# C-bowman/inference-tools

Hardware: AMD Instinct MI355X
Metric: GpRegressor fit+predict wall-time and GFLOP/s at N=16384, d=8; % fp64 MFMA peak (higher is better)
Workload: dtype f64

## Files before the change

### inference-tools_amd/csrc/api.hip

```cpp
#include "api_internal.h"
#include <malloc.h>


thread_local std::string g_create_err;


int lane_streams(gpmi_ctx* c, Lane& L) {
  const size_t index = c->lanes.size() - 1;
  L.owns_stream = index < 2;
  if (!L.owns_stream) L.stream = c->lanes[index % 2].stream;
  if (L.owns_stream) HIPCHK(c, hipStreamCreateWithFlags(&L.stream, hipStreamNonBlocking));
  hipDeviceProp_t prop;
  HIPCHK(c, hipGetDeviceProperties(&prop, c->device));
  c->ncu = prop.multiProcessorCount;
  HIPCHK(c, hipEventCreateWithFlags(&L.ev_la, hipEventDisableTiming));
  HIPCHK(c, hipEventCreateWithFlags(&L.ev_panel, hipEventDisableTiming));
  HIPCHK(c, hipEventCreateWithFlags(&L.ev_join, hipEventDisableTiming));
  HIPCHK(c, hipEventCreateWithFlags(&L.ev_main, hipEventDisableTiming));
  HIPCHK(c, hipEventCreateWithFlags(&L.ev_slice, hipEventDisableTiming));
  return GPMI_OK;
}


bool ensure_masked_pair(gpmi_ctx* c, Lane& L, int k) {
  (void)c;
  return L.sp[k] != nullptr && L.su[k] != nullptr;
}


int lane_masked_streams(gpmi_ctx* c, Lane& L) {
  const int ncu = c->ncu;
  if (ncu < 64 || ncu % 32 != 0) return GPMI_OK;
  for (int k = 0; k < GPMI_NPAIRS; ++k) {
    if (const char* e = std::getenv("GPMI_PANEL_CUS")) {
      const int v = std::atoi(e);
      if (v >= 8 && v <= ncu / 2 && v % 8 == 0) c->pair_cus[k] = v;
    }
    std::vector<uint32_t> panel((size_t)ncu / 32, 0u), upd((size_t)ncu / 32, 0xffffffffu);
    for (int i = 0; i < c->pair_cus[k]; ++i) {
      panel[(size_t)i / 32] |= 1u << (i % 32);
      upd[(size_t)i / 32] &= ~(1u << (i % 32));
    }
    hipError_t e1 = hipExtStreamCreateWithCUMask(&L.sp[k], (uint32_t)panel.size(), panel.data());
    hipError_t e2 = e1 == hipSuccess ? hipExtStreamCreateWithCUMask(&L.su[k], (uint32_t)upd.size(), upd.data()) : e1;
    if (e1 != hipSuccess || e2 != hipSuccess) {
      static bool told = false;
      if (!told) {
        told = true;
        std::fprintf(stderr, "[gpmi] a CU-masked stream pair could not be created (%s): this evaluation lane runs without "
                             "look-ahead and without the flag-ordered tail\n", hipGetErrorString(e1 != hipSuccess ? e1 : e2));
      }
      if (L.sp[k]) (void)hipStreamDestroy(L.sp[k]);
      if (L.su[k]) (void)hipStreamDestroy(L.su[k]);
      L.sp[k] = L.su[k] = nullptr;
      (void)hipGetLastError();
    }
  }
  return GPMI_OK;
}



int lane_alloc(gpmi_ctx* c, Lane& L) {
  if (int rc = lane_streams(c, L)) return rc;
  if (c->lanes.size() == 1 && c->np >= 40 * GPMI_NB)
    if (int rc = lane_masked_streams(c, L)) return rc;
  if (c->lanes.size() == 2 && c->np >= 40 * GPMI_NB) {
    for (int k = 0; k < GPMI_NPAIRS; ++k) {
      L.sp[k] = c->lanes[0].sp[k];
      L.su[k] = c->lanes[0].su[k];
    }
    L.owns_pair = false;
  }
  const int64_t nt = c->np / GPMI_NB;
  HIPCHK(c, hipMalloc(&L.A, sizeof(double) * c->np * c->ld));
  HIPCHK(c, hipMalloc(&L.invD, sizeof(double) * nt * GPMI_NB * GPMI_NB));
  ZERO_SYNC(c, L.invD, sizeof(double) * nt * GPMI_NB * GPMI_NB);
  HIPCHK(c, hipMalloc(&L.vec, sizeof(double) * 4 * c->np));
  HIPCHK(c, hipMalloc(&L.red, sizeof(double) * 2 * RED_SLOTS));
  HIPCHK(c, hipMalloc(&L.info, sizeof(int) * RED_SLOTS));
  HIPCHK(c, hipHostMalloc(&L.h_red, sizeof(double) * 2 * RED_SLOTS));
  HIPCHK(c, hipHostMalloc(&L.h_info, sizeof(int) * RED_SLOTS));
  return GPMI_OK;
}

#define DBG_FREE(msg) do { if (std::getenv("GPMI_DEBUG_FREE")) std::fprintf(stderr, "[free] %s\n", msg); } while (0)
void lane_free(Lane& L) {
  DBG_FREE("lane: sync main stream");
  if (L.stream) (void)hipStreamSynchronize(L.stream);
  DBG_FREE("lane: sync masked streams");
  if (!L.owns_pair)
    for (int k = 0; k < GPMI_NPAIRS; ++k) L.sp[k] = L.su[k] = nullptr;
  for (int k = 0; k < GPMI_NPAIRS; ++k) {
    if (L.sp[k]) (void)hipStreamSynchronize(L.sp[k]);
    if (L.su[k]) (void)hipStreamSynchronize(L.su[k]);
  }
  potrf_flow_free(L);
  DBG_FREE("lane: destroy events");
  if (L.ev_la) (void)hipEventDestroy(L.ev_la);
  if (L.ev_panel) (void)hipEventDestroy(L.ev_panel);
  if (L.ev_join) (void)hipEventDestroy(L.ev_join);
  if (L.ev_main) (void)hipEventDestroy(L.ev_main);
  if (L.ev_slice) (void)hipEventDestroy(L.ev_slice);
  DBG_FREE("lane: destroy masked streams");
  if (L.sp[0] || L.su[0]) {
    static const int pause_ms = [] {
      const char* e = std::getenv("GPMI_DESTROY_PAUSE_MS");
      return e ? std::atoi(e) : 50;
    }();
    std::this_thread::sleep_for(std::chrono::milliseconds(pause_ms));
  }
  for (int k = 0; k < GPMI_NPAIRS; ++k) {
    if (L.sp[k]) (void)hipStreamDestroy(L.sp[k]);
    if (L.su[k]) (void)hipStreamDestroy(L.su[k]);
  }
  DBG_FREE("lane: free buffers");
  if (L.A) (void)hipFree(L.A);
  if (L.B2) (void)hipFree(L.B2);
  if (L.inv2) (void)hipFree(L.inv2);
  if (L.inv2_t) (void)hipFree(L.inv2_t);
  if (L.gws) (void)hipFree(L.gws);
  if (L.invD) (void)hipFree(L.invD);
  if (L.vec) (void)hipFree(L.vec);
  if (L.red) (void)hipFree(L.red);
  if (L.info) (void)hipFree(L.info);
  if (L.h_red) (void)hipHostFree(L.h_red);
  if (L.h_info) (void)hipHostFree(L.h_info);
  DBG_FREE("lane: destroy main stream");
  if (L.stream && L.owns_stream) (void)hipStreamDestroy(L.stream);
  DBG_FREE("lane: done");
  L = Lane();
}

int ensure_lanes(gpmi_ctx* c, size_t count) {
  while (c->lanes.size() < count) {
    c->lanes.emplace_back();
    int rc = lane_alloc(c, c->lanes.back());
    if (rc != GPMI_OK) {
      lane_free(c->lanes.back());
      c->lanes.pop_back();
      return rc;
    }
  }
  return GPMI_OK;
}

void linv_free(LinvState& S);

void free_batch_ws(gpmi_ctx* c) {
  for (double** q : {&c->bA, &c->bInv, &c->bVec, &c->bRed, &c->bMu, &c->bB2, &c->bGws, &c->bGout, &c->bLoo, &c->bQ, &c->bNoise,
                     &c->bMixG, &c->bMixH, &c->bMixW, &c->bMixExtra}) {
    if (*q) (void)hipFree(*q);
    *q = nullptr;
  }
  for (void* q : {(void*)c->bMixP, (void*)c->bInfo, (void*)c->bParams, (void*)c->bSum})
    if (q) (void)hipFree(q);
  c->bMixP = nullptr;
  c->bInfo = nullptr;
  c->bParams = nullptr;
  c->bSum = nullptr;
  for (void* q : {(void*)c->h_bGout, (void*)c->h_bRed, (void*)c->h_bInfo})
    if (q) (void)hipHostFree(q);
  c->h_bGout = c->h_bRed = nullptr;
  c->h_bInfo = nullptr;
  c->bcap = c->bgrad_cap = c->bgrad_ntheta = c->bLoo_cap = c->bNoise_cap = c->bMix_cap = c->bQ_cap = 0;
}

void free_data(gpmi_ctx* c) {
  linv_free(c->linv);
  for (double** q : {&c->mix_g, &c->mix_scratch, &c->mix_zero, &c->Q3}) {
    if (*q) (void)hipFree(*q);
    *q = nullptr;
  }
  c->mix_nk = 0;
  c->q3_cap = 0;
// ... 763 lines not shown
```

### inference-tools_amd/csrc/gpmi_internal.h

```cpp
#pragma once
#include <hip/hip_runtime.h>
#include <cstdint>
#include <string>
#include <vector>

#include "gpmi.h"

constexpr int GPMI_NB = 128;
constexpr int GPMI_MAX_D = 64;
constexpr int GPMI_INFO_FLOW_TIMEOUT = -6;
constexpr int GPMI_NPAIRS = 1;

typedef double d2_t __attribute__((ext_vector_type(2)));
typedef double d4_t __attribute__((ext_vector_type(4)));

static inline int64_t round_up(int64_t v, int64_t m) { return (v + m - 1) / m * m; }

struct KParams {
  int kernel;
  int d;
  double a2;
  double kappa;
  double extra_diag;
  double inv_l2[GPMI_MAX_D];
// ... 16 lines not shown
constexpr int GPMI_MAX_SUM = 4;
struct CovParams : KParams {
  int nk = 0;
  KParams comp[GPMI_MAX_SUM] = {};
  CovParams() : KParams{} {}
  explicit CovParams(const KParams& k) : KParams(k) {}
};

struct ProfSlot {
  hipEvent_t e0, e1;
  int klass;
  double flops, bytes;
};

struct Lane {
  hipStream_t stream = nullptr;
  bool owns_stream = true;
  hipStream_t sp[GPMI_NPAIRS] = {nullptr};
  hipStream_t su[GPMI_NPAIRS] = {nullptr};
  bool owns_pair = true;
  struct EarlyWork {
    bool pending = false;
    const double* y = nullptr;
    const double* mu = nullptr;
    double mu_const = 0.0;
    double* r = nullptr;
    int64_t n = 0, np = 0;
    double* fill[2] = {nullptr, nullptr};
    double* ident = nullptr;
    int64_t ident_ld = 0;
  } early;
  bool identity_ready = false;
  bool pair_checked = false;
  hipEvent_t ev_la = nullptr, ev_panel = nullptr, ev_join = nullptr, ev_main = nullptr, ev_slice = nullptr;
  double* A = nullptr;
  double* invD = nullptr;
  double* B2 = nullptr;
  double* inv2 = nullptr;
  double* inv2_t = nullptr;
  bool inv2_valid = false;
  double* gws = nullptr;
  int64_t gws_doubles = 0;
  double* vec = nullptr;
  double* red = nullptr;
  int* info = nullptr;
  double* h_red = nullptr;
  int* h_info = nullptr;
  void* flow_tasks = nullptr;
  int* flow_off = nullptr;
  int* flow_flags = nullptr;
  int flow_m = 0, flow_nwg = 0, flow_nlists = 0;
  int64_t flow_ntasks = 0;
  double flow_flops_update = 0.0, flow_flops_trsm = 0.0;
};

struct LinvState {
  int64_t m = 0, mp = 0, ldm = 0;
  double* A = nullptr;
  double* At = nullptr;
  double* y = nullptr;
  double* sig2 = nullptr;
  double* zero = nullptr;
  double* K = nullptr;
  double* T = nullptr;
  double* J = nullptr;
  double* J2 = nullptr;
  double* Q = nullptr;
  double* X = nullptr;
  double* invD = nullptr;
  double* inv2 = nullptr;
  double* inv2_t = nullptr;
  double* panel = nullptr;
  double* vec = nullptr;
  double* gws = nullptr;
  int64_t gws_doubles = 0;
};

struct KdeState;
struct gpmi_sgp;

struct gpmi_ctx {
  int device = 0;
  int ncu = 256;
  int pair_cus[GPMI_NPAIRS] = {32};
  std::string err;
  int64_t n = 0, d = 0, np = 0, ld = 0;
  double* x = nullptr;
  double* y = nullptr;
  double* noise = nullptr;
  double* ycov = nullptr;
  std::vector<Lane> lanes;
  bool fitted = false;
  bool lockstep_always = false;
  bool no_flow = false;
  int64_t reserve = 0;
  CovParams fit_params;
  int sum_nk = 0;
  int sum_kinds[GPMI_MAX_SUM] = {};
  double* alpha = nullptr;
  double* Q = nullptr;
  double* Q2 = nullptr;
  int64_t mq_cap = 0;
  double* pts = nullptr;
  double* pvec = nullptr;
  double* trsm_panel = nullptr;
  int64_t trsm_panel_rows = 0;
  double* h_stage = nullptr;
// ... 146 lines not shown
struct BatchShape {
  int count = 1;
  int64_t sMat = 0;
  int64_t sInv = 0;
  int64_t sVec = 0;
};

constexpr int GPMI_MAX_MIX = 4;
void launch_scale_add(hipStream_t s, double* dst, int64_t ldd, const double* src, int64_t lds,
                      const double* gr, const double* gc, int64_t rows, int64_t cols, bool accumulate, int batch = 1,
                      int64_t sD = 0, int64_t sS = 0, int64_t sG = 0);
void launch_add_diag_vec(hipStream_t s, double* A, int64_t ld, const double* noise, double extra, int64_t n,
                         int batch = 1, int64_t sA = 0, const double* extras = nullptr);
void launch_vec_mul(hipStream_t s, const double* a, const double* b, double* out, int64_t n, int batch = 1,
                    int64_t sA = 0, int64_t sB = 0, int64_t sOut = 0);
void launch_mix_rowsum(hipStream_t s, const double* iK, const double* Km, int64_t ld, const double* alpha,
                       const double* g, double* h, int64_t n, int batch = 1, int64_t sMat = 0, int64_t sAlpha = 0,
                       int64_t sG = 0, const double* u = nullptr, int64_t sU = 0, int64_t pair = 0);

enum GemmTiles { TILES_RECT = 0, TILES_LOWER = 1 };
enum GemmOp { OP_SUB = 0, OP_ASSIGN = 1 };
void launch_gemm_nt(hipStream_t s, GemmTiles tiles, GemmOp op, double* C, int64_t ldc,
                    const double* A, int64_t lda, const double* B, int64_t ldb, int ntr, int ntc,
                    int k, unsigned long long* stamp = nullptr, const GemmBatch& bt = GemmBatch());

int64_t gemm_split_point(int64_t T, int ncu, int k);
bool gemm_mixed_launches();
void launch_gemm_nt_split(hipStream_t s, GemmTiles tiles, GemmOp op, double* C, int64_t ldc, const double* A,
                          int64_t lda, const double* B, int64_t ldb, int ntr, int ntc, int k, int64_t nfull,
                          unsigned long long* stamp = nullptr, unsigned long long* stamp_rest = nullptr,
                          int64_t nend = -1);
void launch_gemm_nt_range(hipStream_t s, GemmTiles tiles, GemmOp op, double* C, int64_t ldc, const double* A,
                          int64_t lda, const double* B, int64_t ldb, int ntr, int ntc, int k, int64_t first,
                          int64_t count, unsigned long long* stamp = nullptr);

void launch_gemm(hipStream_t s, GemmTiles tiles, GemmOp op, bool b_kmajor, int kskip, double* C,
                 int64_t ldc, const double* A, int64_t lda, const double* B, int64_t ldb, int ntr,
                 int ntc, int k, unsigned long long* stamp = nullptr, const GemmBatch& bt = GemmBatch());

hipStream_t potrf_first_update_stream(gpmi_ctx* c, Lane& lane, int64_t np, bool allow_lookahead);
void potrf_pair_quiesce(Lane& lane);
void launch_potrf_diag(hipStream_t s, double* Ablk, int64_t ld, double* invD, int* info, int col0,
                       unsigned long long* dbg = nullptr, const BatchShape& bs = BatchShape(), int* pub = nullptr,
                       int pub_val = 0);
void launch_potrf_diag_fault(hipStream_t s, double* Ablk, int64_t ld, const BatchShape& bs = BatchShape());
void potrf_lower_batched(gpmi_ctx* c, hipStream_t s, double* A, int64_t np, int64_t ld, double* invD,
                         int* info, const BatchShape& bs);
void launch_kbuild_square_batched(hipStream_t s, int kernel, const KParams* pdev, int batch, const double* x,
                                  int64_t n, int64_t np, const double* noise, double* A, int64_t ld,
                                  int64_t stride, int d, int64_t noise_stride = 0);
void potrf_lower(gpmi_ctx* c, Lane& lane, double* A, int64_t np, int64_t ld, double* invD,
                 int* info, bool allow_lookahead = true);

bool potrf_flow_enabled(gpmi_ctx* c, Lane& lane, int m);
bool potrf_flow_tail(gpmi_ctx* c, Lane& lane, double* A, int64_t ld, double* invD, int* info, int nt, int t0);
void potrf_flow_free(Lane& lane);

void trsv_forward(gpmi_ctx* c, hipStream_t s, const double* L, int64_t np, int64_t ld,
                  const double* invD, const double* r, double* out, int* err = nullptr,
                  const BatchShape& bs = BatchShape(), bool prefilled = false);
void trsv_backward(gpmi_ctx* c, hipStream_t s, const double* L, int64_t np, int64_t ld,
                   const double* invD, const double* r, double* out, int* err = nullptr,
                   const BatchShape& bs = BatchShape(), bool prefilled = false);
void lane_run_early(Lane& lane, hipStream_t s);
void trsm_identity_batched(hipStream_t s, const double* L, int64_t np, int64_t ld, const double* invD, double* Q,
                           const BatchShape& bs);
constexpr int GPMI_OB = 512;
void build_inv2(hipStream_t s, const double* L, int64_t np, int64_t ld, const double* invD, double* inv2,
                double* tmp);
void trsm_rows_forward(gpmi_ctx* c, hipStream_t s, const double* L, int64_t np, int64_t ld,
                       const double* inv2, double* Q, int64_t mp, bool upper_rhs, double* Qout,
                       double* panel);
void launch_set_identity(hipStream_t s, double* Q, int64_t ld, int64_t np, int batch = 1, int64_t sMat = 0);
void launch_copy(hipStream_t s, const double* src, double* dst, int64_t n);
void launch_copy_rows(hipStream_t s, const double* src, int64_t spitch, double* dst, int64_t dpitch, int64_t width,
                      int64_t height);
void launch_residual(hipStream_t s, const double* y, const double* mu, double mu_const, double* r,
                     int64_t n, int64_t np);
void launch_residual_batched(hipStream_t s, const double* y, const double* mus, const double* mu_consts,
                             double* r, int64_t n, int64_t np, const BatchShape& bs);
void launch_lml_reduce(hipStream_t s, const double* v, const double* L, int64_t ld, int64_t np,
                       double* red, const BatchShape& bs = BatchShape());
void launch_rows_dot(hipStream_t s, const double* Q, int64_t ld, int64_t mp, int64_t np,
                     const double* a, double* out, int batch = 1, int64_t sQ = 0, int64_t sVec = 0);
void launch_rows_sumsq(hipStream_t s, const double* Q, int64_t ld, int64_t mp, int64_t np,
                       double base, double* out, int batch = 1, int64_t sQ = 0, int64_t sVec = 0, double sign = 1.0);

void trsm_rows_backward(gpmi_ctx* c, hipStream_t s, const double* L, int64_t np, int64_t ld,
                        const double* invD, double* Q, int64_t mp, const double* inv2 = nullptr, double* panel = nullptr);

void launch_sd_reduce(hipStream_t s, const KParams& p, const double* x, int64_t n, const double* pts,
                      int64_t m, const double* Kq, int64_t ld, const double* W, int64_t ldw,
                      double scale, double* out);
void launch_grad_rhs(hipStream_t s, const KParams& p, const double* x, int64_t n, int64_t np,
                     const double* pts, int64_t rows_valid, int64_t rows_padded, const double* Kq,
                     int64_t ld, double* G);
void launch_grad_cov(hipStream_t s, const KParams& p, const double* G, int64_t ld, int64_t np,
                     int64_t m, double* cov);
```

### inference-tools_amd/csrc/potrf.hip

```cpp
#include <cstdlib>
#include <type_traits>
#include <utility>
#include <vector>

#include "gpmi_internal.h"
#include "potrf_diag.h"

namespace {

constexpr int NB = GPMI_NB;
using potrf_diag::DIAG_THREADS;

__global__ __launch_bounds__(DIAG_THREADS) void potrf_diag_kernel(double* __restrict__ A, int64_t ld,
                                                         double* __restrict__ invD,
                                                         int* __restrict__ info, int col0,
                                                         unsigned long long* __restrict__ dbg,
                                                         int64_t strideA, int64_t strideInv, int* pub, int pub_val) {
  if (pub && threadIdx.x == 0 && blockIdx.z == 0)
    __hip_atomic_store(pub, pub_val, __ATOMIC_RELAXED, __HIP_MEMORY_SCOPE_AGENT);
  __shared__ potrf_diag::DiagShared sh;
  potrf_diag::potrf_diag_body<false>(A + (int64_t)blockIdx.z * strideA, ld, invD + (int64_t)blockIdx.z * strideInv,
                                     info + blockIdx.z, col0, dbg, sh, potrf_diag::DiagPub());
}

}

namespace {
__global__ void fault_scale_kernel(double* A, int64_t ld, double f, int64_t strideA) {
  A += (int64_t)blockIdx.z * strideA;
  const int r = blockIdx.x, c = threadIdx.x;
  if (c <= r) A[(int64_t)r * ld + c] *= f;
}
}

void launch_potrf_diag_fault(hipStream_t s, double* Ablk, int64_t ld, const BatchShape& bs) {
  static const double fault = [] {
    const char* e = std::getenv("GPMI_FAULT_DIAG_EPS");
    return e ? std::atof(e) : 0.0;
  }();
  if (fault != 0.0)
    hipLaunchKernelGGL(fault_scale_kernel, dim3(NB, 1, (unsigned)bs.count), dim3(NB), 0, s, Ablk, ld, 1.0 + fault,
                       bs.sMat);
}

void launch_potrf_diag(hipStream_t s, double* Ablk, int64_t ld, double* invD, int* info, int col0,
                       unsigned long long* dbg, const BatchShape& bs, int* pub, int pub_val) {
  hipLaunchKernelGGL(potrf_diag_kernel, dim3(1, 1, (unsigned)bs.count), dim3(DIAG_THREADS), 0, s, Ablk, ld, invD,
                     info, col0, dbg, bs.sMat, bs.sInv, pub, pub_val);
  launch_potrf_diag_fault(s, Ablk, ld, bs);
}

namespace {

void factor_panel(gpmi_ctx* c, hipStream_t sp, double* A, int64_t ld, double* invD, int* info, int nt,
                  int J, int Je, int ncu = 0) {
  GemmBatch on;
  on.ncu_hint = ncu;
  on.b_lower_tri = true;
  static const bool trace = std::getenv("GPMI_CHAIN_TRACE") != nullptr;
  auto slot = [&](int tag) { return trace ? prof_stamp_slot(c, 0.0, 0.0, GPMI_PROF_NCLASS + tag) : nullptr; };
  for (int j = J; j < Je; ++j) {
    double* Ajj = A + (int64_t)j * NB * ld + (int64_t)j * NB;
    double* invDj = invD + (int64_t)j * NB * NB;
    const int below = nt - j - 1;
    {
      ProfScope ps(c, sp, GPMI_PROF_PANEL, (double)NB * NB * NB / 3.0 + 2.0 * below * NB * NB * NB,
                   8.0 * NB * NB * (2.0 + 2.0 * below));
      launch_potrf_diag(sp, Ajj, ld, invDj, info, j * NB, slot(0));
      if (below > 0) {
        double* A21 = Ajj + (int64_t)NB * ld;
        launch_gemm_nt(sp, TILES_RECT, OP_ASSIGN, A21, ld, A21, ld, invDj, NB, below, 1, NB, slot(1), on);
      }
    }
    const int pc = Je - j - 1;
    if (below > 0 && pc > 0) {
      double* A21 = Ajj + (int64_t)NB * ld;
      double* C = A21 + NB;
      const double tiles = pc * (pc + 1) / 2.0 + (double)(below - pc) * pc;
      ProfScope ps(c, sp, GPMI_PROF_PANEL, tiles * 2.0 * NB * NB * NB, tiles * 16.0 * NB * NB);
      launch_gemm_nt(sp, TILES_LOWER, OP_SUB, C, ld, A21, ld, A21, ld, below, pc, NB, slot(2));
    }
  }
}

void update_columns(gpmi_ctx* c, hipStream_t s, double* A, int64_t ld, int nt, int t0, int t1, int ka, int ke,
                    int ncu, int64_t slice = 0) {
  const int rows = nt - t0, cols = t1 - t0;
  const int kw = (ke - ka) * NB;
  if (rows <= 0 || cols <= 0 || kw <= 0) return;
  double* P = A + (int64_t)t0 * NB * ld + (int64_t)ka * NB;
  double* C = A + (int64_t)t0 * NB * ld + (int64_t)t0 * NB;
  const int64_t tiles = (int64_t)cols * (cols + 1) / 2 + (int64_t)(rows - cols) * cols - slice;
  const int64_t nfull = gemm_split_point(tiles, ncu, kw);
  static const int64_t BIG_MIN = [] {
    const char* e = std::getenv("GPMI_BIG_MIN");
    return (int64_t)(e ? std::atoi(e) : 384);
  }();
  const bool big = tiles >= BIG_MIN && kw > 128;
  int64_t nmain = big ? nfull : 0;
  if (big && nfull > 0 && nfull < tiles && gemm_mixed_launches()) nmain = tiles;
  unsigned long long* stamp = nullptr;
  unsigned long long* stamp_rest = nullptr;
  if (nmain > 0)
    stamp = prof_stamp_slot(c, (double)nmain * 2.0 * NB * NB * kw, (double)nmain * 16.0 * NB * NB + 8.0 * rows * NB * kw);
  if (tiles > nmain)
    stamp_rest = prof_stamp_slot(c, (double)(tiles - nmain) * 2.0 * NB * NB * kw, (double)(tiles - nmain) * 16.0 * NB * NB,
                                 GPMI_PROF_SYRK_REST);
  if (big)
    launch_gemm_nt_split(s, TILES_LOWER, OP_SUB, C, ld, P, ld, P, ld, rows, cols, kw, nfull, stamp, stamp_rest, tiles);
  else
    launch_gemm_nt_split(s, TILES_LOWER, OP_SUB, C, ld, P, ld, P, ld, rows, cols, kw, nfull, stamp_rest, nullptr, tiles);
}

void update_slice(gpmi_ctx* c, hipStream_t s, double* A, int64_t ld, int nt, int t0, int t1, int ka, int ke,
                  int64_t slice) {
  const int rows = nt - t0, cols = t1 - t0;
  const int kw = (ke - ka) * NB;
  double* P = A + (int64_t)t0 * NB * ld + (int64_t)ka * NB;
  double* C = A + (int64_t)t0 * NB * ld + (int64_t)t0 * NB;
  const int64_t tiles = (int64_t)cols * (cols + 1) / 2 + (int64_t)(rows - cols) * cols;
  unsigned long long* stamp =
      prof_stamp_slot(c, (double)slice * 2.0 * NB * NB * kw, (double)slice * 16.0 * NB * NB + 8.0 * rows * NB * kw,
                      GPMI_PROF_SYRK_SLICE);
  launch_gemm_nt_range(s, TILES_LOWER, OP_SUB, C, ld, P, ld, P, ld, rows, cols, kw, tiles - slice, slice, stamp);
}

int64_t slice_tiles(int rem, int64_t tiles_la, int64_t tiles_main, int kw, int ncu_main, int ncu_panel) {
  static const int PCT = [] {
    const char* e = std::getenv("GPMI_SLICE_PCT");
    return e ? std::atoi(e) : 100;
  }();
  if (PCT <= 0 || kw != 4 * NB) return 0;
  const double tile_us = 64.4 * 2.0;
  const double per_main = tile_us / (2.0 * ncu_main), per_panel = tile_us / (2.0 * ncu_panel);
  static const double CHAIN0 = [] {
    const char* e = std::getenv("GPMI_SLICE_CHAIN_US");
    return e ? std::atof(e) : 146.0;
  }();
  static const double SLOPE = [] {
    const char* e = std::getenv("GPMI_SLICE_CHAIN_SLOPE");
    return e ? std::atof(e) : 6.1;
  }();
  const double chain = CHAIN0 + SLOPE * rem;
  const double su = 20.0 + (double)(tiles_la + tiles_main) * per_main;
  double x = (su - chain) / (per_main + per_panel) * PCT / 100.0;
  const int64_t round = 2 * ncu_panel;
  int64_t n = x > 0 ? (int64_t)(x / round) * round : 0;
  const int64_t safe = tiles_main - (int64_t)8 * rem;
  if (n > safe) n = safe > 0 ? safe / round * round : 0;
  return n;
}

}

bool ensure_masked_pair(gpmi_ctx* c, Lane& L, int k);

namespace {
constexpr int OUTER_TILES = 4;
int lookahead_min() {
  static const int v = [] {
    const char* e = std::getenv("GPMI_LOOKAHEAD_MIN");
    const int x = e ? std::atoi(e) : 52;
    return x > 0 ? x : (1 << 30);
  }();
  return v;
}
}

void potrf_pair_quiesce(Lane& lane) {
  for (int k = 0; k < GPMI_NPAIRS; ++k)
    for (hipStream_t q : {lane.sp[k], lane.su[k]})
      if (q && hipStreamQuery(q) != hipSuccess) {
        (void)hipGetLastError();
        (void)hipStreamSynchronize(q);
      }
  lane.pair_checked = true;
}

hipStream_t potrf_first_update_stream(gpmi_ctx* c, Lane& lane, int64_t np, bool allow_lookahead) {
  const int nt = (int)(np / NB);
  if (!allow_lookahead || nt - OUTER_TILES < lookahead_min() || !ensure_masked_pair(c, lane, 0)) return nullptr;
  return lane.su[0];
}

void potrf_lower(gpmi_ctx* c, Lane& lane, double* A, int64_t np, int64_t ld, double* invD, int* info,
                 bool allow_lookahead) {
  hipStream_t sf = lane.stream;
  const int nt = (int)(np / NB);
  const int OBT = OUTER_TILES;
  const int LOOKAHEAD_MIN = lookahead_min();
  if (!lane.pair_checked) potrf_pair_quiesce(lane);
  lane.pair_checked = false;
  const bool la_ok = allow_lookahead && nt - OBT >= LOOKAHEAD_MIN && ensure_masked_pair(c, lane, 0);
  const bool flow_ok = allow_lookahead;
  if (flow_ok && !(la_ok && nt - OBT >= LOOKAHEAD_MIN) && potrf_flow_enabled(c, lane, nt) &&
      potrf_flow_tail(c, lane, A, ld, invD, info, nt, 0))
    return;
  auto follow = [](hipStream_t waiter, hipStream_t producer, hipEvent_t ev) {
    if (waiter != producer) (void)hipStreamWaitEvent(waiter, ev, 0);
  };
  auto tile0 = [&](int panel) { return panel * OBT < nt ? panel * OBT : nt; };
  const int NP = (nt + OBT - 1) / OBT;
  factor_panel(c, sf, A, ld, invD, info, nt, 0, tile0(1));
  hipStream_t panel_stream = sf;
  hipStream_t main_stream = sf;
  bool sliced = false;
  (void)hipEventRecord(lane.ev_panel, sf);
  (void)hipEventRecord(lane.ev_main, sf);
  if (la_ok && NP > 1 && nt - tile0(1) >= LOOKAHEAD_MIN) lane_run_early(lane, sf);
  for (int p = 0; p + 1 < NP; ++p) {
    const int k0 = tile0(p), k1 = tile0(p + 1);
    const int rem = nt - k1;
    const bool overlap = la_ok && rem >= LOOKAHEAD_MIN;
    hipStream_t su = overlap ? lane.su[0] : sf, sp = overlap ? lane.sp[0] : sf;
    const int ncu = overlap ? c->ncu - c->pair_cus[0] : c->ncu;
    follow(su, panel_stream, lane.ev_panel);
    follow(su, main_stream, lane.ev_main);
    int64_t slice = 0;
    if (overlap) {
      const int k2 = tile0(p + 2);
      update_columns(c, su, A, ld, nt, k1, k2, k0, k1, ncu);
      (void)hipEventRecord(lane.ev_la, su);
      (void)hipStreamWaitEvent(sp, lane.ev_la, 0);
      const int w = k2 - k1, r2 = nt - k2;
      slice = slice_tiles(rem, (int64_t)w * (w + 1) / 2 + (int64_t)(rem - w) * w, (int64_t)r2 * (r2 + 1) / 2,
                          (k1 - k0) * NB, ncu, c->pair_cus[0]);
      if (sliced) (void)hipStreamWaitEvent(su, lane.ev_slice, 0);
      update_columns(c, su, A, ld, nt, k2, nt, k0, k1, ncu, slice);
      (void)hipEventRecord(lane.ev_main, su);
    } else {
      if (sliced) (void)hipStreamWaitEvent(su, lane.ev_slice, 0);
      update_columns(c, su, A, ld, nt, k1, nt, k0, k1, ncu);
      if (flow_ok && potrf_flow_enabled(c, lane, nt - k1) && potrf_flow_tail(c, lane, A, ld, invD, info, nt, k1)) return;
    }
    sliced = false;
    main_stream = su;
    factor_panel(c, sp, A, ld, invD, info, nt, k1, tile0(p + 2), overlap ? c->pair_cus[0] : 0);
    if (overlap) (void)hipEventRecord(lane.ev_panel, sp);
    panel_stream = sp;
    if (slice > 0) {
      update_slice(c, sp, A, ld, nt, tile0(p + 2), nt, k0, k1, slice);
      (void)hipEventRecord(lane.ev_slice, sp);
      sliced = true;
    }
  }
  follow(sf, panel_stream, lane.ev_panel);
  follow(sf, main_stream, lane.ev_main);
  if (sliced) (void)hipStreamWaitEvent(sf, lane.ev_slice, 0);
}

void potrf_lower_batched(gpmi_ctx* c, hipStream_t s, double* A, int64_t np, int64_t ld, double* invD,
                         int* info, const BatchShape& bs) {
  (void)c;
  static const int OBT = [] {
    const char* e = std::getenv("GPMI_BATCH_OUTER");
    const int v = e ? std::atoi(e) : 4;
    return v > 0 ? v : 1;
  }();
  const int nt = (int)(np / NB);
  GemmBatch inplace{bs.count, bs.sMat, bs.sMat, bs.sInv};
  inplace.b_lower_tri = true;
  const GemmBatch upd{bs.count, bs.sMat, bs.sMat, bs.sMat};
  static const bool left = [] {
    const char* e = std::getenv("GPMI_BATCH_LEFT");
    return !e || std::atoi(e) != 0;
  }();
  for (int J = 0; J < nt; J += OBT) {
    const int Je = (J + OBT < nt) ? J + OBT : nt;
    for (int j = J; j < Je; ++j) {
      double* Ajj = A + (int64_t)j * NB * ld + (int64_t)j * NB;
      double* invDj = invD + (int64_t)j * NB * NB;
      const int below = nt - j - 1;
      if (left && j > J) {
        const double* P = A + (int64_t)j * NB * ld + (int64_t)J * NB;
        launch_gemm_nt(s, TILES_LOWER, OP_SUB, Ajj, ld, P, ld, P, ld, nt - j, 1, (j - J) * NB, nullptr, upd);
      }
      launch_potrf_diag(s, Ajj, ld, invDj, info, j * NB, nullptr, bs);
      if (below > 0) {
        double* A21 = Ajj + (int64_t)NB * ld;
        launch_gemm_nt(s, TILES_RECT, OP_ASSIGN, A21, ld, A21, ld, invDj, NB, below, 1, NB, nullptr, inplace);
        const int pc = Je - j - 1;
        if (!left && pc > 0)
          launch_gemm_nt(s, TILES_LOWER, OP_SUB, A21 + NB, ld, A21, ld, A21, ld, below, pc, NB, nullptr, upd);
      }
    }
    const int rest = nt - Je;
    if (rest > 0) {
      double* P = A + (int64_t)Je * NB * ld + (int64_t)J * NB;
      double* C = A + (int64_t)Je * NB * ld + (int64_t)Je * NB;
      launch_gemm_nt(s, TILES_LOWER, OP_SUB, C, ld, P, ld, P, ld, rest, rest, (Je - J) * NB, nullptr, upd);
// ... 4 lines not shown
```

### inference-tools_amd/csrc/potrf_flow.hip

```cpp
#include <algorithm>
#include <cstdio>
#include <cstdlib>
#include <mutex>
#include <tuple>
#include <vector>

#include "gemm_tiles.h"
#include "potrf_diag.h"

using namespace gemm_tiles;

namespace {

constexpr int NB = GPMI_NB;
constexpr int OBT = 4;
int env_int(const char* name, int dflt) {
  const char* e = std::getenv(name);
  return e ? std::atoi(e) : dflt;
}
const int FLOW_NEAR_D = env_int("GPMI_FLOW_NEAR_D", 3);
const int FLOW_NEAR_WGS = (env_int("GPMI_FLOW_NEAR_WGS", 32) + 7) / 8 * 8;
constexpr int FT_T = 0, FT_U = 1, FT_Z = 2, FT_ZS = 3;
const int FLOW_SPLIT = env_int("GPMI_FLOW_SPLIT", 1);
const int FLOW_QUARTER = env_int("GPMI_FLOW_QUARTER", 0);
const int FLOW_URGENT = env_int("GPMI_FLOW_URGENT", 3);

struct FlowTask {
  uint8_t type, s, fadd, pad;
  uint16_t i, j, k, pad2;
};
static_assert(sizeof(FlowTask) == 12, "FlowTask layout");

constexpr int FL_DDONE = 0, FL_ABORT = 32, FL_T0 = 48, FL_STATS = 64, FL_ROWCNT = 96, FL_INVROW = 128, FL_LCNT = 384;
__host__ __device__ inline int flow_f_off(int m) { return FL_LCNT + ((m + 31) / 32) * 32; }
__host__ __device__ inline int flow_owner_off(int m) { return flow_f_off(m) + ((m * m + 31) / 32) * 32; }
inline int flow_flag_ints(int m, int nwg) { return flow_owner_off(m) + nwg; }
constexpr int FLOW_MAX_LISTS = 1536;
constexpr int FLOW_MAX_WGS = 512;
constexpr unsigned long long FLOW_GRACE_TICKS = 5000;

struct FlowArgs {
  double* A;
  const double* invD;
  int64_t ld;
  int m;
  const FlowTask* tasks;
  const int* off;
  int nlists;
  int* flags;
  int* info;
  unsigned long long* stamp;
  unsigned long long* stats;
  unsigned long long* trace;
  int fault;
};

__device__ __forceinline__ bool flow_ready(const FlowTask& t, const int* __restrict__ fl, int m) {
  const int* Lcnt = fl + FL_LCNT;
  const int* F = fl + flow_f_off(m);
  if (t.type == FT_T) return flow_ld(fl + FL_DDONE) >= t.k + 1 && flow_ld(F + t.i * m + t.k) == 4 * t.k;
// ... 301 lines not shown
  const bool pair = w >= 24;
  int r0, r1;
  if (pair) {
    r0 = 2 * (w - 24);
    r1 = r0 + 1;
  } else {
    int n = w, i = 1, j = 0;
    for (;;) {
      const bool pair_tile = (i & 1) && j == i - 1;
      if (!pair_tile) {
        if (n == 0) break;
        --n;
      }
      if (++j == i) {
        ++i;
        j = 0;
      }
    }
    r0 = i;
    r1 = j;
  }
  r0 = __builtin_amdgcn_readfirstlane(r0);
  r1 = __builtin_amdgcn_readfirstlane(r1);
  const d4_t t0 = *reinterpret_cast<const d4_t*>(T + (int64_t)(16 * r0 + fr) * g.ld + 16 * c + 4 * fk);
  const d4_t t1 = *reinterpret_cast<const d4_t*>(T + (int64_t)(16 * r1 + fr) * g.ld + 16 * c + 4 * fk);
  const bool tile_wave = pair ? (c >= 3 && c <= 5) : c == 3;
  int ti = r0, tj = r1;
  if (pair) {
    ti = c == 3 ? r0 : r1;
    tj = c == 4 ? r1 : r0;
  }
  d4_t acc = {0.0, 0.0, 0.0, 0.0};
  double* cp = C + (int64_t)(16 * ti + fk) * g.ld + 16 * tj + fr;
  if (tile_wave) {
#pragma unroll
    for (int r = 0; r < 4; ++r) acc[r] = cp[(int64_t)4 * r * g.ld];
  }
  *reinterpret_cast<d4_t*>(&Ts[fr * CF_APITCH + 16 * c + 4 * fk]) = t0;
  *reinterpret_cast<d4_t*>(&Ts[16 * CF_APITCH + fr * CF_APITCH + 16 * c + 4 * fk]) = t1;
  __syncthreads();
  if (tid == 0) {
    __hip_atomic_fetch_add(fl + FL_ROWCNT + r0, 1, __ATOMIC_RELAXED, __HIP_MEMORY_SCOPE_AGENT);
    __hip_atomic_fetch_add(fl + FL_ROWCNT + r1, 1, __ATOMIC_RELAXED, __HIP_MEMORY_SCOPE_AGENT);
  }
  const int row_target = potrf_diag::DIAG_INVERSE * (g.k + 1);
  const int readers_target = CC_READERS * (g.k + 1);
  const double* xa = Xs + (pair ? (ti == r0 ? 0 : 1) : 0) * 16 * CF_PITCH + fr * CF_PITCH + 2 * fk;
  const double* xb = Xs + (pair ? (tj == r0 ? 0 : 1) : 1) * 16 * CF_PITCH + fr * CF_PITCH + 2 * fk;
  bool readers_seen = false;
#pragma unroll
  for (int row = 0; row < NB / 16; ++row) {
    if (row == c || row == 7 - c) {
      const int strip = row == c ? 0 : 1;
      {
        int spins = 0;
        while (flow_ld(fl + FL_INVROW + 32 * row) < row_target) {
          __builtin_amdgcn_s_sleep(2);
          if ((++spins & 63) == 0 && flow_ld(abortw)) break;
          if (spins > FLOW_SPIN_LIMIT) {
            give_up();
            break;
          }
        }
        __builtin_amdgcn_fence(__ATOMIC_ACQUIRE, "agent");
      }
      const double* brow = g.invD + (int64_t)(16 * row + fr) * NB + 4 * fk;
      d4_t b[NB / 16];
#pragma unroll
      for (int s = 0; s <= row; ++s) b[s] = *reinterpret_cast<const d4_t*>(brow + 16 * s);
      d4_t x = {0.0, 0.0, 0.0, 0.0};
      const double* ts = Ts + strip * 16 * CF_APITCH + fr * CF_APITCH + 4 * fk;
#pragma unroll
      for (int s = 0; s <= row; ++s) {
        const d4_t a = *reinterpret_cast<const d4_t*>(ts + 16 * s);
#pragma unroll
        for (int q = 0; q < 4; ++q) x = __builtin_amdgcn_mfma_f64_16x16x4f64(a[q], b[s][q], x, 0, 0, 0);
      }
      double* xo = Xs + strip * 16 * CF_PITCH + fk * CF_PITCH + 16 * row + fr;
#pragma unroll
      for (int r = 0; r < 4; ++r) xo[4 * r * CF_PITCH] = x[r];
      asm volatile("s_waitcnt lgkmcnt(0)" ::: "memory");
      if (lane == 0) __hip_atomic_fetch_add(xs_cnt + row, 1, __ATOMIC_RELAXED, __HIP_MEMORY_SCOPE_WORKGROUP);
      if (pair) {
        if (!readers_seen) {
          int spins = 0;
          while (flow_ld(fl + FL_ROWCNT + r0) < readers_target || flow_ld(fl + FL_ROWCNT + r1) < readers_target) {
            __builtin_amdgcn_s_sleep(2);
            if ((++spins & 63) == 0 && flow_ld(abortw)) break;
            if (spins > FLOW_SPIN_LIMIT) {
              give_up();
              break;
            }
          }
          readers_seen = true;
        }
        double* o = T + (int64_t)(16 * (strip ? r1 : r0) + fk) * g.ld + 16 * row + fr;
#pragma unroll
        for (int r = 0; r < 4; ++r) o[(int64_t)4 * r * g.ld] = x[r];
      }
    }
    if (tile_wave) {
      int polls = 0;
      while (__hip_atomic_load(xs_cnt + row, __ATOMIC_RELAXED, __HIP_MEMORY_SCOPE_WORKGROUP) < 2) {
        __builtin_amdgcn_s_sleep(1);
        if ((++polls & 1023) == 0 && flow_ld(abortw)) break;
        if (polls > (1 << 24)) {
          give_up();
          break;
        }
      }
      asm volatile("" ::: "memory");
#pragma unroll
      for (int st = 2 * row; st < 2 * row + 2; ++st) {
        const d2_t av = *reinterpret_cast<const d2_t*>(xa + 8 * st);
        const d2_t bv = *reinterpret_cast<const d2_t*>(xb + 8 * st);
#pragma unroll
        for (int h = 0; h < 2; ++h) acc = __builtin_amdgcn_mfma_f64_16x16x4f64(av[h], bv[h], acc, 0, 0, 1);
      }
    }
  }
  if (tile_wave) {
    if (g.trace && w == 0) g.trace[2] = __builtin_amdgcn_s_memrealtime();
#pragma unroll
    for (int r = 0; r < 4; ++r) cp[(int64_t)4 * r * g.ld] = acc[r];
    if (g.trace && w == 0 && lane == 0) {
      asm volatile("s_waitcnt vmcnt(0)" ::: "memory");
      g.trace[3] = __builtin_amdgcn_s_memrealtime();
    }
  }
}
// ... 627 lines not shown
```

Before: 55320.

## Fuse panel diagonal factorization with below-diagonal TRSM in one flag-synchronized kernel

Adds a panel-column kernel in which block 0 factors the diagonal tile and publishes inverse rows through device flags. The remaining blocks spin on those flags and apply the inverse to the below-diagonal tiles with fp64 MFMA, replacing a separate diag launch followed by a GEMM. The shared colblock helper is factored out of the flow kernel, and the slice-tile chain model gets different default constants when fused. The intent is to remove a launch and serialization on the panel critical path, at the cost of cross-block spin-waiting and reliance on co-residency of the blocks.

```diff
diff --git a/inference-tools_amd/csrc/api.hip b/inference-tools_amd/csrc/api.hip
--- a/inference-tools_amd/csrc/api.hip
+++ b/inference-tools_amd/csrc/api.hip
@@ -18,6 +18,8 @@
   HIPCHK(c, hipEventCreateWithFlags(&L.ev_join, hipEventDisableTiming));
   HIPCHK(c, hipEventCreateWithFlags(&L.ev_main, hipEventDisableTiming));
   HIPCHK(c, hipEventCreateWithFlags(&L.ev_slice, hipEventDisableTiming));
+  HIPCHK(c, hipMalloc(&L.panel_flags, sizeof(int) * GPMI_PANEL_FL_INTS));
+  ZERO_SYNC(c, L.panel_flags, sizeof(int) * GPMI_PANEL_FL_INTS);
   return GPMI_OK;
 }
 
@@ -121,6 +123,7 @@
   if (L.inv2_t) (void)hipFree(L.inv2_t);
   if (L.gws) (void)hipFree(L.gws);
   if (L.invD) (void)hipFree(L.invD);
+  if (L.panel_flags) (void)hipFree(L.panel_flags);
   if (L.vec) (void)hipFree(L.vec);
   if (L.red) (void)hipFree(L.red);
   if (L.info) (void)hipFree(L.info);
diff --git a/inference-tools_amd/csrc/gpmi_internal.h b/inference-tools_amd/csrc/gpmi_internal.h
--- a/inference-tools_amd/csrc/gpmi_internal.h
+++ b/inference-tools_amd/csrc/gpmi_internal.h
@@ -92,7 +92,10 @@
   int flow_m = 0, flow_nwg = 0, flow_nlists = 0;
   int64_t flow_ntasks = 0;
   double flow_flops_update = 0.0, flow_flops_trsm = 0.0;
-};
+  int* panel_flags = nullptr;
+  unsigned panel_seq = 0;
+};
+constexpr int GPMI_PANEL_FL_INVROW = 0, GPMI_PANEL_FL_ABORT = 256, GPMI_PANEL_FL_INTS = 288;
 
 struct LinvState {
   int64_t m = 0, mp = 0, ldm = 0;
@@ -345,6 +348,10 @@
 void potrf_lower(gpmi_ctx* c, Lane& lane, double* A, int64_t np, int64_t ld, double* invD,
                  int* info, bool allow_lookahead = true);
 
+bool potrf_panel_fused(gpmi_ctx* c, Lane& lane);
+void launch_panel_column(Lane& lane, hipStream_t s, double* Akk, int64_t ld, double* invD, int* info, int col0, int below,
+                         int ncu, unsigned long long* dbg = nullptr, unsigned long long* stamp = nullptr);
+
 bool potrf_flow_enabled(gpmi_ctx* c, Lane& lane, int m);
 bool potrf_flow_tail(gpmi_ctx* c, Lane& lane, double* A, int64_t ld, double* invD, int* info, int nt, int t0);
 void potrf_flow_free(Lane& lane);
diff --git a/inference-tools_amd/csrc/potrf.hip b/inference-tools_amd/csrc/potrf.hip
--- a/inference-tools_amd/csrc/potrf.hip
+++ b/inference-tools_amd/csrc/potrf.hip
@@ -52,11 +52,12 @@
 
 namespace {
 
-void factor_panel(gpmi_ctx* c, hipStream_t sp, double* A, int64_t ld, double* invD, int* info, int nt,
+void factor_panel(gpmi_ctx* c, Lane& lane, hipStream_t sp, double* A, int64_t ld, double* invD, int* info, int nt,
                   int J, int Je, int ncu = 0) {
   GemmBatch on;
   on.ncu_hint = ncu;
   on.b_lower_tri = true;
+  const bool fused = potrf_panel_fused(c, lane);
   static const bool trace = std::getenv("GPMI_CHAIN_TRACE") != nullptr;
   auto slot = [&](int tag) { return trace ? prof_stamp_slot(c, 0.0, 0.0, GPMI_PROF_NCLASS + tag) : nullptr; };
   for (int j = J; j < Je; ++j) {
@@ -66,8 +67,13 @@
     {
       ProfScope ps(c, sp, GPMI_PROF_PANEL, (double)NB * NB * NB / 3.0 + 2.0 * below * NB * NB * NB,
                    8.0 * NB * NB * (2.0 + 2.0 * below));
-      launch_potrf_diag(sp, Ajj, ld, invDj, info, j * NB, slot(0));
-      if (below > 0) {
+      if (below > 0 && fused) {
+        unsigned long long* s0 = slot(0);
+        launch_panel_column(lane, sp, Ajj, ld, invDj, info, j * NB, below, ncu > 0 ? ncu : c->ncu, s0, slot(1));
+      } else {
+        launch_potrf_diag(sp, Ajj, ld, invDj, info, j * NB, slot(0));
+      }
+      if (below > 0 && !fused) {
         double* A21 = Ajj + (int64_t)NB * ld;
         launch_gemm_nt(sp, TILES_RECT, OP_ASSIGN, A21, ld, A21, ld, invDj, NB, below, 1, NB, slot(1), on);
       }
@@ -125,7 +131,7 @@
   launch_gemm_nt_range(s, TILES_LOWER, OP_SUB, C, ld, P, ld, P, ld, rows, cols, kw, tiles - slice, slice, stamp);
 }
 
-int64_t slice_tiles(int rem, int64_t tiles_la, int64_t tiles_main, int kw, int ncu_main, int ncu_panel) {
+int64_t slice_tiles(int rem, int64_t tiles_la, int64_t tiles_main, int kw, int ncu_main, int ncu_panel, bool fused) {
   static const int PCT = [] {
     const char* e = std::getenv("GPMI_SLICE_PCT");
     return e ? std::atoi(e) : 100;
@@ -133,14 +139,16 @@
   if (PCT <= 0 || kw != 4 * NB) return 0;
   const double tile_us = 64.4 * 2.0;
   const double per_main = tile_us / (2.0 * ncu_main), per_panel = tile_us / (2.0 * ncu_panel);
-  static const double CHAIN0 = [] {
+  static const double CHAIN0_ENV = [] {
     const char* e = std::getenv("GPMI_SLICE_CHAIN_US");
-    return e ? std::atof(e) : 146.0;
-  }();
-  static const double SLOPE = [] {
+    return e ? std::atof(e) : -1.0;
+  }();
+  static const double SLOPE_ENV = [] {
     const char* e = std::getenv("GPMI_SLICE_CHAIN_SLOPE");
-    return e ? std::atof(e) : 6.1;
-  }();
+    return e ? std::atof(e) : -1.0;
+  }();
+  const double CHAIN0 = CHAIN0_ENV >= 0.0 ? CHAIN0_ENV : (fused ? 93.0 : 146.0);
+  const double SLOPE = SLOPE_ENV >= 0.0 ? SLOPE_ENV : (fused ? 5.17 : 6.1);
   const double chain = CHAIN0 + SLOPE * rem;
   const double su = 20.0 + (double)(tiles_la + tiles_main) * per_main;
   double x = (su - chain) / (per_main + per_panel) * PCT / 100.0;
@@ -201,7 +209,7 @@
   };
   auto tile0 = [&](int panel) { return panel * OBT < nt ? panel * OBT : nt; };
   const int NP = (nt + OBT - 1) / OBT;
-  factor_panel(c, sf, A, ld, invD, info, nt, 0, tile0(1));
+  factor_panel(c, lane, sf, A, ld, invD, info, nt, 0, tile0(1));
   hipStream_t panel_stream = sf;
   hipStream_t main_stream = sf;
   bool sliced = false;
@@ -224,7 +232,7 @@
       (void)hipStreamWaitEvent(sp, lane.ev_la, 0);
       const int w = k2 - k1, r2 = nt - k2;
       slice = slice_tiles(rem, (int64_t)w * (w + 1) / 2 + (int64_t)(rem - w) * w, (int64_t)r2 * (r2 + 1) / 2,
-                          (k1 - k0) * NB, ncu, c->pair_cus[0]);
+                          (k1 - k0) * NB, ncu, c->pair_cus[0], potrf_panel_fused(c, lane));
       if (sliced) (void)hipStreamWaitEvent(su, lane.ev_slice, 0);
       update_columns(c, su, A, ld, nt, k2, nt, k0, k1, ncu, slice);
       (void)hipEventRecord(lane.ev_main, su);
@@ -235,7 +243,7 @@
     }
     sliced = false;
     main_stream = su;
-    factor_panel(c, sp, A, ld, invD, info, nt, k1, tile0(p + 2), overlap ? c->pair_cus[0] : 0);
+    factor_panel(c, lane, sp, A, ld, invD, info, nt, k1, tile0(p + 2), overlap ? c->pair_cus[0] : 0);
     if (overlap) (void)hipEventRecord(lane.ev_panel, sp);
     panel_stream = sp;
     if (slice > 0) {
diff --git a/inference-tools_amd/csrc/potrf_colblock.h b/inference-tools_amd/csrc/potrf_colblock.h
--- /dev/null
+++ b/inference-tools_amd/csrc/potrf_colblock.h
@@ -0,0 +1,47 @@
+#pragma once
+#include "gemm_tiles.h"
+#include "potrf_diag.h"
+
+namespace potrf_colblock {
+
+using gemm_tiles::flow_ld;
+using gemm_tiles::FLOW_SPIN_LIMIT;
+constexpr int NB = GPMI_NB;
+
+__device__ __forceinline__ bool flag_reached(int seen, int target) { return (int)((unsigned)seen - (unsigned)target) >= 0; }
+
+template <class GiveUp>
+__device__ __forceinline__ void wait_inv_row(const int* rowflag, int target, const int* abortw, GiveUp&& give_up) {
+  int spins = 0;
+  while (!flag_reached(flow_ld(rowflag), target)) {
+    __builtin_amdgcn_s_sleep(2);
+    if ((++spins & 63) == 0 && flow_ld(abortw)) break;
+    if (spins > FLOW_SPIN_LIMIT) {
+      give_up();
+      break;
+    }
+  }
+  __builtin_amdgcn_fence(__ATOMIC_ACQUIRE, "agent");
+}
+
+__device__ __forceinline__ void load_inv_rowblock(const double* inv, int pitch, int row, int fr, int fk,
+                                                  d4_t (&b)[NB / 16]) {
+  const double* brow = inv + (int64_t)(16 * row + fr) * pitch + 4 * fk;
+#pragma unroll
+  for (int s = 0; s < NB / 16; ++s)
+    if (s <= row) b[s] = *reinterpret_cast<const d4_t*>(brow + 16 * s);
+}
+template <class ASlab>
+__device__ __forceinline__ d4_t colblock_sums(int row, ASlab&& a_slab, const d4_t (&b)[NB / 16]) {
+  d4_t x = {0.0, 0.0, 0.0, 0.0};
+#pragma unroll
+  for (int s = 0; s < NB / 16; ++s)
+    if (s <= row) {
+      const d4_t a = a_slab(s);
+#pragma unroll
+      for (int q = 0; q < 4; ++q) x = __builtin_amdgcn_mfma_f64_16x16x4f64(a[q], b[s][q], x, 0, 0, 0);
+    }
+  return x;
+}
+
+}
diff --git a/inference-tools_amd/csrc/potrf_flow.hip b/inference-tools_amd/csrc/potrf_flow.hip
--- a/inference-tools_amd/csrc/potrf_flow.hip
+++ b/inference-tools_amd/csrc/potrf_flow.hip
@@ -6,6 +6,7 @@
 #include <vector>
 
 #include "gemm_tiles.h"
+#include "potrf_colblock.h"
 #include "potrf_diag.h"
 
 using namespace gemm_tiles;
@@ -413,30 +414,12 @@
   for (int row = 0; row < NB / 16; ++row) {
     if (row == c || row == 7 - c) {
       const int strip = row == c ? 0 : 1;
-      {
-        int spins = 0;
-        while (flow_ld(fl + FL_INVROW + 32 * row) < row_target) {
-          __builtin_amdgcn_s_sleep(2);
-          if ((++spins & 63) == 0 && flow_ld(abortw)) break;
-          if (spins > FLOW_SPIN_LIMIT) {
-            give_up();
-            break;
-          }
-        }
-        __builtin_amdgcn_fence(__ATOMIC_ACQUIRE, "agent");
-      }
-      const double* brow = g.invD + (int64_t)(16 * row + fr) * NB + 4 * fk;
+      potrf_colblock::wait_inv_row(fl + FL_INVROW + 32 * row, row_target, abortw, give_up);
+      const double* ts = Ts + strip * 16 * CF_APITCH + fr * CF_APITCH + 4 * fk;
       d4_t b[NB / 16];
-#pragma unroll
-      for (int s = 0; s <= row; ++s) b[s] = *reinterpret_cast<const d4_t*>(brow + 16 * s);
-      d4_t x = {0.0, 0.0, 0.0, 0.0};
-      const double* ts = Ts + strip * 16 * CF_APITCH + fr * CF_APITCH + 4 * fk;
-#pragma unroll
-      for (int s = 0; s <= row; ++s) {
-        const d4_t a = *reinterpret_cast<const d4_t*>(ts + 16 * s);
-#pragma unroll
-        for (int q = 0; q < 4; ++q) x = __builtin_amdgcn_mfma_f64_16x16x4f64(a[q], b[s][q], x, 0, 0, 0);
-      }
+      potrf_colblock::load_inv_rowblock(g.invD, NB, row, fr, fk, b);
+      const d4_t x =
+          potrf_colblock::colblock_sums(row, [&](int s) { return *reinterpret_cast<const d4_t*>(ts + 16 * s); }, b);
       double* xo = Xs + strip * 16 * CF_PITCH + fk * CF_PITCH + 16 * row + fr;
 #pragma unroll
       for (int r = 0; r < 4; ++r) xo[4 * r * CF_PITCH] = x[r];
diff --git a/inference-tools_amd/csrc/potrf_panel.hip b/inference-tools_amd/csrc/potrf_panel.hip
--- /dev/null
+++ b/inference-tools_amd/csrc/potrf_panel.hip
@@ -0,0 +1,135 @@
+#include <cstdlib>
+
+#include "gpmi_internal.h"
+#include "potrf_colblock.h"
+#include "potrf_diag.h"
+
+namespace {
+
+constexpr int NB = GPMI_NB;
+constexpr int INV_PITCH = NB + 6;
+using gemm_tiles::flow_ld;
+
+struct PanelColArgs {
+  double* Akk;
+  double* invD;
+  int64_t ld;
+  int* info;
+  int col0;
+  unsigned long long* dbg;
+  unsigned long long* stamp;
+  int* flags;
+  unsigned seq;
+  int below;
+};
+
+__global__ __launch_bounds__(potrf_diag::DIAG_THREADS) void panel_column_kernel(PanelColArgs g) {
+  __shared__ potrf_diag::DiagShared sh;
+  if (blockIdx.x == 0) {
+    potrf_diag::DiagPub pub;
+    pub.rows = g.flags + GPMI_PANEL_FL_INVROW;
+    pub.base = (int)(potrf_diag::DIAG_INVERSE * g.seq);
+    potrf_diag::potrf_diag_body<true>(g.Akk, g.ld, g.invD, g.info, g.col0, g.dbg, sh, pub);
+    return;
+  }
+  const int w = (int)blockIdx.x - 1, W = (int)gridDim.x - 1;
+  const int tid = threadIdx.x, lane = tid & 63, r = __builtin_amdgcn_readfirstlane((int)(tid >> 6));
+  const int fr = lane & 15, fk = lane >> 4;
+  const int* rows = g.flags + GPMI_PANEL_FL_INVROW;
+  int* abortw = g.flags + GPMI_PANEL_FL_ABORT;
+  auto give_up = [&]() {
+    if (lane == 0) {
+      __hip_atomic_store(abortw, 1, __ATOMIC_RELAXED, __HIP_MEMORY_SCOPE_AGENT);
+      if (g.info) atomicCAS(g.info, 0, GPMI_INFO_FLOW_TIMEOUT);
+    }
+  };
+  if (g.stamp && w == 0 && tid == 0) g.stamp[0] = __builtin_amdgcn_s_memrealtime();
+  double* inv_lds = reinterpret_cast<double*>(&sh);
+  int* seen = reinterpret_cast<int*>(inv_lds + NB * INV_PITCH);
+  static_assert(sizeof(double) * NB * INV_PITCH + sizeof(int) <= sizeof(potrf_diag::DiagShared), "the worker's LDS");
+  if (tid == 0) *seen = 0;
+  __syncthreads();
+  const int row_target = (int)(potrf_diag::DIAG_INVERSE * (g.seq + 1u));
+  auto fetch = [&](int i, d4_t (&t)[NB / 16]) {
+    const double* trow = g.Akk + (int64_t)(i + 1) * NB * g.ld + (int64_t)(16 * r + fr) * g.ld + 4 * fk;
+#pragma unroll
+    for (int s = 0; s < NB / 16; ++s) t[s] = *reinterpret_cast<const d4_t*>(trow + 16 * s);
+  };
+  auto store_block = [&](int i, int c, const d4_t& x) {
+    double* out = g.Akk + (int64_t)(i + 1) * NB * g.ld + (int64_t)(16 * r + fk) * g.ld + fr;
+#pragma unroll
+    for (int q = 0; q < 4; ++q) out[(int64_t)4 * q * g.ld + 16 * c] = x[q];
+  };
+  d4_t a[NB / 16], an[NB / 16];
+  fetch(w, a);
+  if (w + W < g.below) fetch(w + W, an);
+#pragma unroll
+  for (int c = 0; c < NB / 16; ++c) {
+    d4_t b[NB / 16];
+    if (r == c) {
+      potrf_colblock::wait_inv_row(rows + 32 * c, row_target, abortw, give_up);
+      potrf_colblock::load_inv_rowblock(g.invD, NB, c, fr, fk, b);
+      double* brow = inv_lds + (16 * c + fr) * INV_PITCH + 4 * fk;
+#pragma unroll
+      for (int s = 0; s <= c; ++s) *reinterpret_cast<d4_t*>(brow + 16 * s) = b[s];
+      asm volatile("s_waitcnt lgkmcnt(0)" ::: "memory");
+      if (lane == 0) __hip_atomic_store(seen, c + 1, __ATOMIC_RELAXED, __HIP_MEMORY_SCOPE_WORKGROUP);
+    } else {
+      int polls = 0;
+      while (__hip_atomic_load(seen, __ATOMIC_RELAXED, __HIP_MEMORY_SCOPE_WORKGROUP) <= c) {
+        __builtin_amdgcn_s_sleep(1);
+        if ((++polls & 1023) == 0 && flow_ld(abortw)) break;
+        if (polls > (1 << 25)) {
+          give_up();
+          break;
+        }
+      }
+      asm volatile("" ::: "memory");
+      potrf_colblock::load_inv_rowblock(inv_lds, INV_PITCH, c, fr, fk, b);
+    }
+    store_block(w, c, potrf_colblock::colblock_sums(c, [&](int s) { return a[s]; }, b));
+  }
+  if (w + W < g.below) {
+    __syncthreads();
+    for (int i = w + W; i < g.below; i += W) {
+#pragma unroll
+      for (int s = 0; s < NB / 16; ++s) a[s] = an[s];
+      if (i + W < g.below) fetch(i + W, an);
+#pragma unroll
+      for (int c = 0; c < NB / 16; ++c) {
+        d4_t b[NB / 16];
+        potrf_colblock::load_inv_rowblock(inv_lds, INV_PITCH, c, fr, fk, b);
+        store_block(i, c, potrf_colblock::colblock_sums(c, [&](int s) { return a[s]; }, b));
+        __builtin_amdgcn_sched_barrier(0);
+      }
+    }
+  }
+  if (g.stamp && tid == 0) {
+    asm volatile("s_waitcnt vmcnt(0)" ::: "memory");
+    g.stamp[8 + (__builtin_amdgcn_s_getreg(((4 - 1) << 11) | 20) & 7)] = __builtin_amdgcn_s_memrealtime();
+  }
+}
+
+}
+
+bool potrf_panel_fused(gpmi_ctx* c, Lane& lane) {
+  static const bool on = [] {
+    const char* e = std::getenv("GPMI_PANEL_FUSED");
+    return !e || std::atoi(e) != 0;
+  }();
+  return on && !c->no_flow && lane.panel_flags != nullptr;
+}
+
+void launch_panel_column(Lane& lane, hipStream_t s, double* Akk, int64_t ld, double* invD, int* info, int col0, int below,
+                         int ncu, unsigned long long* dbg, unsigned long long* stamp) {
+  static const int clamp = [] {
+    const char* e = std::getenv("GPMI_PANEL_WORKERS");
+    return e ? std::atoi(e) : 0;
+  }();
+  int W = ncu - 1 < below ? ncu - 1 : below;
+  if (clamp > 0 && W > clamp) W = clamp;
+  if (W < 1) W = 1;
+  PanelColArgs g{Akk, invD, ld, info, col0, dbg, stamp, lane.panel_flags, lane.panel_seq++, below};
+  hipLaunchKernelGGL(panel_column_kernel, dim3(1u + (unsigned)W), dim3(potrf_diag::DIAG_THREADS), 0, s, g);
+  launch_potrf_diag_fault(s, Akk, ld);
+}
```

New measurement: 55980 (median of 6 runs). +1.2%, better.
